# kasirershahartau/tissue_image_processing

Measured on AMD Instinct MI355X. Metric: frames/sec end-to-end (2048^2, z=30), higher is better.
Workload: dtype f32(f16x3)

## Files before the change

tissue_image_processing_amd/csrc/tip_core.hip:

```cpp
#include "tip_internal.h"
#include <algorithm>
#include <cmath>
#include <cstdlib>
#include <map>
#include <mutex>

namespace tip {

static thread_local Ctx *g_ctx = nullptr;
static thread_local int g_requested_device = 0;

static int ctx_create(int device)
{
    Ctx *c = new Ctx();
    c->device = device;
    hipError_t e = hipSetDevice(device);
    if (e != hipSuccess) {
        c->err = std::string("hipSetDevice failed: ") + hipGetErrorString(e);
        g_ctx = c;
        return TIP_ERR_HIP;
    }
    {
        const char *pr = getenv("TIP_STREAM_PRIORITY");
        int lo = 0, hi = 0;
// ... 61 lines not shown
    }
    c.pool.push_back({p, bytes, true});
    return p;
}

void *pinned_scratch(size_t bytes)
{
    Ctx &c = ctx();
    if (c.pin_bytes >= bytes && c.pin_buf) return c.pin_buf;
    if (c.pin_buf) { (void)hipHostFree(c.pin_buf); c.pin_buf = nullptr; c.pin_bytes = 0; }
    const size_t want = bytes + (bytes >> 2) + 4096;
    void *p = nullptr;
    if (hipHostMalloc(&p, want, hipHostMallocDefault) != hipSuccess) {
        (void)hipGetLastError();
        fail(TIP_ERR_NOMEM, "hipHostMalloc(%zu) failed", want);
        return nullptr;
    }
    c.pin_buf = p;
    c.pin_bytes = want;
    return p;
}

void ws_free(void *p)
{
    Ctx &c = ctx();
    for (auto &b : c.pool)
        if (b.p == p) { b.used = false; return; }
}

void prof_begin(const char *name)
{
    Ctx &c = ctx();
    if (!c.prof) return;
    ProfRec r;
    r.name = name;
    if (c.free_events.size() >= 2) {
        r.e0 = c.free_events.back(); c.free_events.pop_back();
        r.e1 = c.free_events.back(); c.free_events.pop_back();
    } else {
        (void)hipEventCreate(&r.e0);
        (void)hipEventCreate(&r.e1);
    }
    (void)hipEventRecord(r.e0, c.stream);
    c.recs.push_back(r);
}

void prof_end()
{
    Ctx &c = ctx();
    if (!c.prof) return;
    (void)hipEventRecord(c.recs.back().e1, c.stream);
}

namespace {
Tuning g_tuning;
std::once_flag g_tuning_once;
std::mutex g_tuning_mu;

bool tuning_assign(Tuning &t, const char *name, const char *value)
{
    const Tuning def;
    const bool unset = !value || !*value;
    auto flag = [&](int &field, int dflt) { field = unset ? dflt : (strcmp(value, "0") != 0 ? 1 : 0); };
    auto num = [&](int &field, int dflt) { field = unset ? dflt : atoi(value); };
    auto pair = [&](int &a, int &b, int da, int db) {
        a = da; b = db;
        if (!unset) sscanf(value, "%d,%d", &a, &b);
    };
    const std::string n(name ? name : "");
    if (n == "TIP_WS_TIES") {
        if (unset) t.ws_ties = def.ws_ties;
        else t.ws_ties = (!strcmp(value, "fast") || !strcmp(value, "0")) ? 0 : 1;
    }
    else if (n == "TIP_WS_OPEN") pair(t.ws_open_a, t.ws_open_b, def.ws_open_a, def.ws_open_b);
    else if (n == "TIP_WS_NO_SKIP") flag(t.ws_no_skip, 0);
    else if (n == "TIP_WS_DEBUG") flag(t.ws_debug, 0);
    else if (n == "TIP_WS_NO_ENDGAME") flag(t.ws_no_endgame, 0);
    else if (n == "TIP_WS_NO_WIDE") flag(t.ws_no_wide, 0);
    else if (n == "TIP_PROJECT_GENERIC") flag(t.project_generic, 0);
    else if (n == "TIP_PROJECT_UNFUSED_PREBLUR") flag(t.project_unfused_preblur, 0);
    else if (n == "TIP_PROJECT_UNFUSED_MASK") flag(t.project_unfused_mask, 0);
    else if (n == "TIP_PROJECT_EXACT_SCORE") flag(t.project_exact_score, 0);
    else if (n == "TIP_PROJECT_DEBUG") flag(t.project_debug, 0);
    else if (n == "TIP_UNET_TILE8") num(t.unet_tile8, def.unet_tile8);
    else if (n == "TIP_UF_ONE_LEVEL") flag(t.uf_one_level, 0);
    else if (n == "TIP_UNET_SPB") num(t.unet_spb, def.unet_spb);
    else if (n == "TIP_UNET_MFMA") { num(t.unet_mfma, def.unet_mfma); if (t.unet_mfma != 32) t.unet_mfma = 16; }
    else if (n == "TIP_UNET_XCD_MAP") flag(t.unet_xcd_map, 1);
    else if (n == "TIP_UNET_FIRST") {
        if (unset || !strcmp(value, "mfma")) t.unet_first_mfma = def.unet_first_mfma;
        else t.unet_first_mfma = !strcmp(value, "valu") ? 0 : std::max(atoi(value), 0);
    }
    else if (n == "TIP_UNET_TAIL_UNFUSED") flag(t.unet_tail_unfused, 0);
    else if (n == "TIP_MB_SMALL") num(t.mb_small, def.mb_small);
    else if (n == "TIP_MB_BATCH") num(t.mb_batch, def.mb_batch);
    else return false;
    return true;
}

const char *const TUNING_NAMES[] = {"TIP_WS_TIES", "TIP_WS_OPEN", "TIP_WS_NO_SKIP", "TIP_WS_DEBUG", "TIP_WS_NO_ENDGAME", "TIP_WS_NO_WIDE",
                                    "TIP_PROJECT_GENERIC", "TIP_PROJECT_UNFUSED_PREBLUR", "TIP_PROJECT_UNFUSED_MASK",
                                    "TIP_PROJECT_EXACT_SCORE", "TIP_PROJECT_DEBUG", "TIP_UNET_TILE8", "TIP_UNET_TAIL_UNFUSED", "TIP_UNET_XCD_MAP", "TIP_UNET_SPB", "TIP_UNET_MFMA", "TIP_UNET_FIRST", "TIP_UF_ONE_LEVEL", "TIP_MB_SMALL", "TIP_MB_BATCH"};

void tuning_from_env()
{
    for (const char *name : TUNING_NAMES)
        if (const char *e = getenv(name)) tuning_assign(g_tuning, name, e);
}
}

const Tuning &tuning()
{
    std::call_once(g_tuning_once, tuning_from_env);
    return g_tuning;
}

int make_taps(Taps &t, const double *w, int n)
{
    if (n <= 0 || n > 255 || !(n & 1)) return fail(TIP_ERR_ARG, "tap count %d must be odd and <= 255", n);
    for (int i = 1; i <= n / 2; i++)
        if (fabs(w[n / 2 + i] - w[n / 2 - i]) > 2.220446049250313e-16)
            return fail(TIP_ERR_UNSUPPORTED, "only symmetric kernels (scipy's symmetric correlate1d branch)");
    memset(&t, 0, sizeof t);
    for (int i = 0; i < n; i++) t.w[i] = w[i];
    t.n = n;
    return TIP_OK;
}

static double np_pairwise_sum(const double *a, long n)
{
    if (n < 8) {
        double r = 0.0;
        for (long i = 0; i < n; i++) r += a[i];
        return r;
    } else if (n <= 128) {
        double r[8];
        long i;
        for (i = 0; i < 8; i++) r[i] = a[i];
        for (i = 8; i < n - (n % 8); i += 8)
            for (int k = 0; k < 8; k++) r[k] += a[i + k];
        double res = ((r[0] + r[1]) + (r[2] + r[3])) + ((r[4] + r[5]) + (r[6] + r[7]));
        for (; i < n; i++) res += a[i];
        return res;
    }
    long n2 = n / 2;
    n2 -= n2 % 8;
    return np_pairwise_sum(a, n2) + np_pairwise_sum(a + n2, n - n2);
}

int libm_taps(double sigma, double truncate, double *w, int cap)
{
    long radius = (long)(truncate * sigma + 0.5);
    long n = 2 * radius + 1;
    if (n > cap) return -1;
    double s2 = sigma * sigma;
    for (long i = 0; i < n; i++) {
        double x = (double)(i - radius);
        w[i] = exp(-0.5 / s2 * (x * x));
    }
    double sum = np_pairwise_sum(w, n);
    for (long i = 0; i < n; i++) w[i] = w[i] / sum;
    return (int)n;
}

}

using namespace tip;

extern "C" {

int tip_version(void) { return 100; }

int tip_device_count(void)
{
    int n = 0;
    if (hipGetDeviceCount(&n) != hipSuccess) return 0;
    return n;
}

int tip_init(int device)
{
    if (g_ctx) {
        if (g_ctx->device == device && g_ctx->stream) return TIP_OK;
        tip_shutdown();
    }
// ... 190 lines not shown
```

tissue_image_processing_amd/csrc/tip_corr_f16.h:

```cpp
#pragma once
#include "tip_corr.h"
#include "tip_unet_conv.h"

namespace tip {

constexpr int HF_TO = 256, HF_LN = 32, HF_NW = 4;
typedef float hf_f32x4 __attribute__((ext_vector_type(4)));

struct HfScale {
    float s, inv;
};
__device__ __forceinline__ HfScale hf_scale(const float *clip_p95, const int *clip_has)
{
    const float c = (clip_has && *clip_has && *clip_p95 > 0.f) ? *clip_p95 : 1.f;
    const int e = min(max((int)((__float_as_uint(c) >> 23) & 0xffu) - 127, -60), 100);
    HfScale h;
    h.s = __uint_as_float((unsigned)(127 + 13 - e) << 23);
    h.inv = __uint_as_float((unsigned)(127 - 13 + e - 17) << 23);
    return h;
}

template <int AXIS, int R8>
__global__ void __launch_bounds__(HF_NW * 64, 2) k_corr_long_f16(const float *__restrict__ in, float *__restrict__ out, int Z, int Y, int X,
                                                                  TapsF taps, const float *__restrict__ clip_p95, const int *__restrict__ clip_has,
                                                                  int *__restrict__ range_flag, int tiles_ln, int tiles_pos, int xcd_bands)
{
    constexpr int r = 8 * R8, NPOS = HF_TO + 2 * r, S = R8 + 2;
    constexpr int PCH = (NPOS / 8) | 1, PITCH = PCH * 8;
    constexpr int WROWS = 2 * S + 3;
    extern __shared__ __attribute__((aligned(16))) unsigned char hf_smem[];
    _Float16 *sB_hi = reinterpret_cast<_Float16 *>(hf_smem), *sB_lo = sB_hi + HF_LN * PITCH;
    uint4 *sW_hi = reinterpret_cast<uint4 *>(sB_lo + HF_LN * PITCH), *sW_lo = sW_hi + WROWS * 8;
    const int tid = threadIdx.x, lane = tid & 63, wave = __builtin_amdgcn_readfirstlane(tid >> 6);
    const int z = blockIdx.y;
    int lx, py;
    if (AXIS == 2 && xcd_bands) {
        const int b = blockIdx.x, k = b & 7, j = b >> 3;
        py = j % tiles_pos;
        lx = k + 8 * (j / tiles_pos);
    } else {
        lx = blockIdx.x % tiles_ln;
        py = blockIdx.x / tiles_ln;
    }
    const int p0 = py * HF_TO, l0 = lx * HF_LN;
    const long P = (long)Y * X;
    const float *src = in + (long)z * P;
    const HfScale sc = hf_scale(clip_p95, clip_has);

    for (int idx = tid; idx < WROWS * 8; idx += HF_NW * 64) {
        const int up = (idx >> 3) - 3, c = idx & 7;
        f16x8 hi, lo;
#pragma unroll
        for (int e = 0; e < 8; ++e) {
            const int d = 8 * up - c + e, ad = d - r < 0 ? r - d : d - r;
            const float w = (d >= 0 && d <= 2 * r) ? taps.w[r - ad] * 131072.f : 0.f;
            hi[e] = (_Float16)w;
            lo[e] = (_Float16)((w - (float)hi[e]) * 2048.f);
        }
        sW_hi[idx] = __builtin_bit_cast(uint4, hi);
        sW_lo[idx] = __builtin_bit_cast(uint4, lo);
    }
    float vmax = 0.f;
    auto split8 = [&](const float (&v)[8], int line, int g) {
        f16x8 hi, lo;
#pragma unroll
        for (int e = 0; e < 8; ++e) {
            const float vs = v[e] * sc.s;
            vmax = fmax_raw(vmax, vs);
            hi[e] = (_Float16)vs;
            lo[e] = (_Float16)__builtin_fmaf(vs - (float)hi[e], 2048.f, fminf(vs * 1.329227995784916e36f, 5.9604644775390625e-8f));
        }
        *reinterpret_cast<uint4 *>(sB_hi + line * PITCH + 8 * g) = __builtin_bit_cast(uint4, hi);
        *reinterpret_cast<uint4 *>(sB_lo + line * PITCH + 8 * g) = __builtin_bit_cast(uint4, lo);
    };
    constexpr int NG = NPOS / 8;
    if (AXIS == 2) {
        constexpr int NIT = (HF_LN * NG + HF_NW * 64 - 1) / (HF_NW * 64);
        hf_f32x4 ld[NIT][2];
        const bool vec = (X & 3) == 0;
        constexpr int DL = (HF_NW * 64) / NG, DG = (HF_NW * 64) - DL * NG;
        const int line_0 = tid / NG, g_0 = tid - line_0 * NG;
        int uline[NIT], ug[NIT];
        {
            int line = line_0, g = g_0;
#pragma unroll
            for (int it = 0; it < NIT; ++it) {
                uline[it] = line;
                ug[it] = g;
                line += DL;
                g += DG;
                if (g >= NG) { g -= NG; ++line; }
            }
        }
#pragma unroll
        for (int it = 0; it < NIT; ++it) {
            const int line = uline[it], g = ug[it];
            const float *row = src + (long)min(l0 + min(line, HF_LN - 1), Y - 1) * X;
            const int x0 = p0 - r + 8 * g;
            if (vec && x0 >= 0 && x0 + 8 <= X) {
                ld[it][0] = *reinterpret_cast<const hf_f32x4 *>(row + x0);
                ld[it][1] = *reinterpret_cast<const hf_f32x4 *>(row + x0 + 4);
            } else {
                ld[it][0] = hf_f32x4{row[clampi(x0, 0, X - 1)], row[clampi(x0 + 1, 0, X - 1)], row[clampi(x0 + 2, 0, X - 1)], row[clampi(x0 + 3, 0, X - 1)]};
                ld[it][1] = hf_f32x4{row[clampi(x0 + 4, 0, X - 1)], row[clampi(x0 + 5, 0, X - 1)], row[clampi(x0 + 6, 0, X - 1)], row[clampi(x0 + 7, 0, X - 1)]};
            }
        }
#pragma unroll
        for (int it = 0; it < NIT; ++it) {
            const int line = uline[it], g = ug[it];
            if (line < HF_LN) {
                const float v[8] = {ld[it][0][0], ld[it][0][1], ld[it][0][2], ld[it][0][3], ld[it][1][0], ld[it][1][1], ld[it][1][2], ld[it][1][3]};
                split8(v, line, g);
            }
        }
    } else {
        constexpr int NIT = (NG * (HF_LN / 4) + HF_NW * 64 - 1) / (HF_NW * 64);
        hf_f32x4 ld[NIT][8];
        const int lq = tid & 7;
        const int xq = l0 + 4 * lq;
        const bool vec = (X & 3) == 0 && xq + 4 <= X;
        if (vec) {
#pragma unroll
            for (int it = 0; it < NIT; ++it) {
                const int g = min(it * (HF_NW * 8) + (tid >> 3), NG - 1), y0 = p0 - r + 8 * g;
#pragma unroll
                for (int e = 0; e < 8; ++e) ld[it][e] = *reinterpret_cast<const hf_f32x4 *>(src + (long)clampi(y0 + e, 0, Y - 1) * X + xq);
            }
        } else {
#pragma unroll
            for (int it = 0; it < NIT; ++it) {
                const int g = min(it * (HF_NW * 8) + (tid >> 3), NG - 1), y0 = p0 - r + 8 * g;
#pragma unroll
                for (int e = 0; e < 8; ++e) {
                    const float *row = src + (long)clampi(y0 + e, 0, Y - 1) * X;
                    ld[it][e] = hf_f32x4{row[min(xq, X - 1)], row[min(xq + 1, X - 1)], row[min(xq + 2, X - 1)], row[min(xq + 3, X - 1)]};
                }
            }
        }
#pragma unroll
        for (int it = 0; it < NIT; ++it) {
            const int g = it * (HF_NW * 8) + (tid >> 3);
            if (g < NG) {
                float v[8];
#pragma unroll
                for (int e = 0; e < 8; ++e) v[e] = ld[it][e].x;
                split8(v, 4 * lq, g);
#pragma unroll
                for (int e = 0; e < 8; ++e) v[e] = ld[it][e].y;
                split8(v, 4 * lq + 1, g);
#pragma unroll
                for (int e = 0; e < 8; ++e) v[e] = ld[it][e].z;
                split8(v, 4 * lq + 2, g);
#pragma unroll
                for (int e = 0; e < 8; ++e) v[e] = ld[it][e].w;
                split8(v, 4 * lq + 3, g);
            }
        }
    }
    if (!(vmax < 40000.f)) atomicOr(range_flag, 8);
    __syncthreads();

    const int i = lane & 31, h = lane >> 5;
    const int len = AXIS == 1 ? Y : X;
    if (p0 + wave * 64 >= len) return;
    const _Float16 *bh = sB_hi + i * PITCH + wave * 64 + 8 * h, *bl = sB_lo + i * PITCH + wave * 64 + 8 * h;
    const int wrow0 = (h - (i >> 3) + 3) * 8 + (i & 7);
    f32x16 thh[2], tm[2], ahh[2], am[2];
#pragma unroll
    for (int t = 0; t < 2; ++t)
#pragma unroll
        for (int q = 0; q < 16; ++q) { thh[t][q] = 0.f; tm[t][q] = 0.f; ahh[t][q] = 0.f; am[t][q] = 0.f; }
    uint4 fh[3], fl[3];
    auto mm = [](const uint4 &wf, const uint4 &sf, const f32x16 &c) -> f32x16 {
        if (AXIS == 1) return __builtin_amdgcn_mfma_f32_32x32x16_f16(__builtin_bit_cast(f16x8, wf), __builtin_bit_cast(f16x8, sf), c, 0, 0, 0);
        return __builtin_amdgcn_mfma_f32_32x32x16_f16(__builtin_bit_cast(f16x8, sf), __builtin_bit_cast(f16x8, wf), c, 0, 0, 0);
    };
    auto flush = [&](int t) {
#pragma unroll
        for (int q = 0; q < 16; q += 2) {
            f32x2 x = f32x2{thh[t][q], thh[t][q + 1]} + f32x2{ahh[t][q], ahh[t][q + 1]};
            f32x2 y = f32x2{tm[t][q], tm[t][q + 1]} + f32x2{am[t][q], am[t][q + 1]};
            asm volatile("" : "+v"(x), "+v"(y));
            thh[t][q] = x[0]; thh[t][q + 1] = x[1];
            tm[t][q] = y[0]; tm[t][q + 1] = y[1];
            ahh[t][q] = 0.f; ahh[t][q + 1] = 0.f;
            am[t][q] = 0.f; am[t][q + 1] = 0.f;
        }
    };
#pragma unroll
    for (int s = 0; s < S + 2; ++s) {
        const uint4 sh = *reinterpret_cast<const uint4 *>(bh + 16 * s), sl = *reinterpret_cast<const uint4 *>(bl + 16 * s);
        if (s < S) {
            fh[s % 3] = sW_hi[wrow0 + 16 * s];
            fl[s % 3] = sW_lo[wrow0 + 16 * s];
            ahh[0] = mm(fh[s % 3], sh, ahh[0]);
            am[0] = mm(fh[s % 3], sl, am[0]);
            am[0] = mm(fl[s % 3], sh, am[0]);
            if ((s & 1) == 1 || s == S - 1) flush(0);
        }
        if (s >= 2) {
            const int k = (s - 2) % 3;
            ahh[1] = mm(fh[k], sh, ahh[1]);
            am[1] = mm(fh[k], sl, am[1]);
            am[1] = mm(fl[k], sh, am[1]);
            if (((s - 2) & 1) == 1 || s == S + 1) flush(1);
        }
        __builtin_amdgcn_sched_barrier(0);
    }
    float *dst = out + (long)z * P;
#pragma unroll
    for (int t = 0; t < 2; ++t) {
        const int o0 = p0 + wave * 64 + 32 * t;
#pragma unroll
        for (int q = 0; q < 16; ++q) {
            const int rr = (q & 3) + 8 * (q >> 2) + 4 * h;
            const float val = __builtin_fmaf(tm[t][q], 4.8828125e-4f, thh[t][q]) * sc.inv;
            if (AXIS == 1) {
                const int yy = o0 + rr, xx = l0 + i;
                if (yy < Y && xx < X) dst[(long)yy * X + xx] = val;
            } else {
                const int yy = l0 + rr, xx = o0 + i;
                if (yy < Y && xx < X) dst[(long)yy * X + xx] = val;
            }
        }
    }
}

}
```

tissue_image_processing_amd/csrc/tip_internal.h:

```cpp
#pragma once
#include <hip/hip_runtime.h>
#include <cstdarg>
#include <cstdint>
#include <cstdio>
#include <cstring>
#include <string>
#include <vector>
#include "../../include/tissue_hip.h"

namespace tip {

struct ProfRec { const char *name; hipEvent_t e0, e1; };

struct Ctx {
    int device = -1;
    hipStream_t stream = nullptr;
    std::string err;
    struct Block { void *p; size_t bytes; bool used; };
    std::vector<Block> pool;
    int last_ws_labels = 0;
    long last_ws_other = 0;
    hipEvent_t edge_event = nullptr;
    void *prep_ws = nullptr;
    unsigned *unet_status = nullptr;
    int *unet_status_host = nullptr;
    void *pin_buf = nullptr;
    size_t pin_bytes = 0;
    bool prof = false;
    std::vector<ProfRec> recs;
    std::vector<hipEvent_t> free_events;
};

Ctx &ctx();
int fail(int code, const char *fmt, ...);
int launch_check(const char *what);
void *ws_alloc(size_t bytes);
void *pinned_scratch(size_t bytes);
void ws_free(void *p);

struct WsGuard {
    std::vector<void *> ptrs;
    template <typename T> T *get(size_t count) {
        void *p = ws_alloc(count * sizeof(T) ? count * sizeof(T) : 16);
        if (p) ptrs.push_back(p);
        return (T *)p;
    }
    ~WsGuard() { for (void *p : ptrs) ws_free(p); }
};

struct Staging {
    WsGuard ws;
    int rc = TIP_OK;
    struct Out { void *host; const void *dev; size_t bytes; };
    std::vector<Out> outs;

    bool hip(hipError_t e, const char *what)
    {
        if (e != hipSuccess && !rc) rc = fail(TIP_ERR_HIP, "%s failed: %s", what, hipGetErrorString(e));
        return !rc;
    }
    template <typename T> T *scratch(size_t count)
    {
        if (rc) return nullptr;
        T *d = ws.get<T>(count);
        if (!d) rc = TIP_ERR_NOMEM;
        return d;
    }
    template <typename T> T *in(const T *host, size_t count)
    {
        T *d = host ? scratch<T>(count) : nullptr;
        if (d && count) hip(hipMemcpyAsync(d, host, count * sizeof(T), hipMemcpyHostToDevice, ctx().stream), "hipMemcpyAsync (upload)");
        return d;
    }
    template <typename T> T *out(T *host, size_t count, bool zero = false)
    {
        T *d = host ? scratch<T>(count) : nullptr;
        if (d && zero && count) hip(hipMemsetAsync(d, 0, count * sizeof(T), ctx().stream), "hipMemsetAsync");
        if (d) outs.push_back({host, d, count * sizeof(T)});
        return d;
    }
    template <typename T> void set_count(const T *dev, size_t count)
    {
        for (Out &o : outs)
            if (o.dev == dev && count * sizeof(T) < o.bytes) o.bytes = count * sizeof(T);
    }
    int finish()
    {
        for (const Out &o : outs)
            if (o.bytes && !hip(hipMemcpyAsync(o.host, o.dev, o.bytes, hipMemcpyDeviceToHost, ctx().stream), "hipMemcpyAsync (download)")) break;
        if (!rc) hip(hipStreamSynchronize(ctx().stream), "hipStreamSynchronize");
        return rc;
    }
};

void prof_begin(const char *name);
void prof_end();

struct Tuning {
    int ws_ties = 1;
    int ws_open_a = -1, ws_open_b = -1;
    int ws_no_skip = 0;
    int ws_debug = 0;
    int ws_no_endgame = 0, ws_no_wide = 0;
    int project_generic = 0, project_unfused_preblur = 0, project_unfused_mask = 0;
    int project_exact_score = 0, project_debug = 0;
    int unet_tail_unfused = 0;
    int unet_xcd_map = 1;
    int unet_spb = 3;
    int unet_mfma = 32;
    int unet_first_mfma = 1;
    int uf_one_level = 0;
    int mb_small = -1;
    int mb_batch = -1;
    int unet_tile8 = -1;
};
const Tuning &tuning();

#define TIP_HIP(call)                                                                             \
    do {                                                                                          \
        hipError_t e__ = (call);                                                                  \
        if (e__ != hipSuccess)                                                                    \
            return tip::fail(TIP_ERR_HIP, "%s failed: %s (%s:%d)", #call, hipGetErrorString(e__), \
                             __FILE__, __LINE__);                                                 \
    } while (0)

#define TIP_LAUNCH(name, kernel, grid, block, shmem, ...)                                  \
    do {                                                                                   \
        tip::prof_begin(name);                                                             \
        hipLaunchKernelGGL(kernel, grid, block, shmem, tip::ctx().stream, __VA_ARGS__);    \
        tip::prof_end();                                                                   \
        hipError_t e__ = hipGetLastError();                                                \
        if (e__ != hipSuccess)                                                             \
            return tip::fail(TIP_ERR_HIP, "launch %s: %s", name, hipGetErrorString(e__));  \
    } while (0)

static inline int cdiv(long a, long b) { return (int)((a + b - 1) / b); }

struct Taps {
    double w[256];
    int n;
};
struct TapsF {
    float w[256];
    int n;
};

int make_taps(Taps &t, const double *w, int n);
int libm_taps(double sigma, double truncate, double *w, int cap);
int correlate1d_dev(const void *in, void *out, int dtype, int Z, int Y, int X, int axis, const Taps &t, int force);

constexpr int OF_F64_AS_U16 = 5;
int optical_flow_tvl1_dev(const void *ref, const void *mov, int dtype, int y, int x, float attachment, float tightness,
                          int num_warp, int num_iter, double tol, float *flow_out, int32_t *warps_host, int cap);

int scan_i32_dev(const int32_t *in, int32_t *out, int n);

}
```

tissue_image_processing_amd/csrc/tip_project.hip:

```cpp
#include "tip_slide.h"
#include "tip_preblur.h"
#include "tip_corr.h"
#include "tip_corr_f16.h"
#include "tip_manifold.h"
#include "tip_project_binned.h"
#include <algorithm>
#include <atomic>
#include <cstdlib>

namespace tip {

struct ClipInfo {
    double p95d;
    float p95;
    int has;
};

template <typename T>
__device__ __forceinline__ T wave_inclusive_scan(T v, int lane)
{
    for (int d = 1; d < 64; d <<= 1) {
        const T o = __shfl_up(v, d, 64);
        if (lane >= d) v += o;
    }
// ... 270 lines not shown
        for (int c = cx; c < cx + 8 + 2 * MASK_R; ++c) { za = min(za, (int)cmin[ty][c]); zb = max(zb, (int)cmax[ty][c]); }
        za = max(za - MASK_ZR, 0); zb = min(zb + MASK_ZR, Zs - 1);
    }
    float mx[MAXC][8];
#pragma unroll
    for (int c = 0; c < MAXC; ++c)
#pragma unroll
        for (int k = 0; k < 8; ++k) mx[c][k] = 0.f;
    for (int z = zaB; z <= zbB; ++z) {
        float(*yb)[FT_W] = ybuf[(z - zaB) & 1];
        const float *Tz = sT + z * Zs;
        for (int i = t; i < FT_Y * FT_W; i += 256) {
            const int r = i / FT_W, c = i - r * FT_W;
            float val = 0.f;
            if (z >= (int)cmin[r][c] - MASK_ZR && z <= (int)cmax[r][c] + MASK_ZR)
                val = (float)tap_sum<MASK_R>([&](int j) { return (double)Tz[zs[r + j][c]]; }, taps.w);
            yb[r][c] = val;
        }
        __syncthreads();
        if (live && z >= za && z <= zb) {
            float v[8 + 2 * MASK_R];
#pragma unroll
            for (int i = 0; i < (8 + 2 * MASK_R) / 4; ++i) {
                const float4 f = *reinterpret_cast<const float4 *>(&yb[ty][cx + 4 * i]);
                v[4 * i] = f.x; v[4 * i + 1] = f.y; v[4 * i + 2] = f.z; v[4 * i + 3] = f.w;
            }
            float m[8];
#pragma unroll
            for (int k = 0; k < 8; ++k) m[k] = (float)tap_sum<MASK_R>([&](int j) { return (double)v[k + j]; }, taps.w);
#pragma unroll
            for (int c = 0; c < MAXC; ++c) {
                if (c < C && ((chan_mask >> c) & 1u)) {
                    const uint16_t *ip = img + ((long)c * Zfull + zlo + z) * P + (long)gy * X + gx;
                    unsigned short pix[8];
                    if (gx + 8 <= X && (X & 7) == 0) {
                        const uint4 u = *reinterpret_cast<const uint4 *>(ip);
                        pix[0] = u.x & 0xffff; pix[1] = u.x >> 16; pix[2] = u.y & 0xffff; pix[3] = u.y >> 16;
                        pix[4] = u.z & 0xffff; pix[5] = u.z >> 16; pix[6] = u.w & 0xffff; pix[7] = u.w >> 16;
                    } else {
#pragma unroll
                        for (int k = 0; k < 8; ++k) pix[k] = gx + k < X ? ip[k] : 0;
                    }
#pragma unroll
                    for (int k = 0; k < 8; ++k) {
                        const float pr = airy_offset((float)pix[k], airy) * m[k];
                        mx[c][k] = pr > mx[c][k] ? pr : mx[c][k];
                    }
                }
            }
        }
    }
    if (live) {
#pragma unroll
        for (int c = 0; c < MAXC; ++c)
            if (c < C && ((chan_mask >> c) & 1u))
#pragma unroll
                for (int k = 0; k < 8; ++k)
                    if (gx + k < X) proj[(long)c * P + (long)gy * X + gx + k] = (double)mx[c][k];
    }
}

static int cu_count()
{
    static int cus = 0;
    if (!cus) {
        hipDeviceProp_t prop;
        cus = hipGetDeviceProperties(&prop, ctx().device) == hipSuccess && prop.multiProcessorCount > 0 ? prop.multiProcessorCount : 256;
    }
    return cus;
}

static TapsF taps_f32(const double *w, int n)
{
    TapsF f;
    f.n = n;
    for (int i = 0; i < 256; ++i) f.w[i] = i < n ? (float)w[i] : 0.f;
    return f;
}

template <int AXIS>
static int launch_f16(const float *in, float *out, int Zs, int Y, int X, const TapsF &t, const ClipInfo *clip, int *range_flag)
{
    if (t.n != 241 || !clip || !range_flag) return fail(TIP_ERR_ARG, "f16 score pass: %d taps (241 only) or no clip value / range flag", t.n);
    constexpr int R8 = 15, NPOS = HF_TO + 16 * R8, PITCH = ((NPOS / 8) | 1) * 8, WROWS = 2 * (R8 + 2) + 3;
    const size_t lds = (size_t)2 * HF_LN * PITCH * 2 + (size_t)2 * WROWS * 8 * 16;
    auto k = k_corr_long_f16<AXIS, R8>;
    static std::atomic<unsigned> attr_done[64];
    const int dev = ctx().device >= 0 && ctx().device < 64 ? ctx().device : 0;
    if (!(attr_done[dev].load(std::memory_order_acquire) & (1u << AXIS))) {
        TIP_HIP(hipFuncSetAttribute((const void *)k, hipFuncAttributeMaxDynamicSharedMemorySize, (int)lds));
        attr_done[dev].fetch_or(1u << AXIS, std::memory_order_release);
    }
    const int tiles_ln = cdiv(AXIS == 1 ? X : Y, HF_LN), tiles_pos = cdiv(AXIS == 1 ? Y : X, HF_TO);
    if ((long)tiles_ln * tiles_pos > 0x7fffffffL || Zs > 65535) return fail(TIP_ERR_ARG, "f16 score pass: grid too large");
    const dim3 grid((unsigned)(tiles_ln * tiles_pos), (unsigned)Zs);
    const int xcd_bands = (AXIS == 2 && tiles_ln % 8 == 0) ? 1 : 0;
    TIP_LAUNCH(AXIS == 1 ? "score_fast_y" : "score_fast_x", k, grid, dim3(HF_NW * 64), lds, in, out, Zs, Y, X, t, &clip->p95, &clip->has, range_flag,
               tiles_ln, tiles_pos, xcd_bands);
    return TIP_OK;
}

#define CERT_EPS (96.0f * 5.9604644775390625e-8f)
__device__ __forceinline__ float cert_abs(const ClipInfo *clip)
{
    return (clip && clip->has) ? clip->p95 * 5.684341886080802e-14f + 1e-30f : 1e-30f;
}

__global__ void __launch_bounds__(256) k_argmax_certify(const float *__restrict__ score, int Z, long P, int *__restrict__ best_z,
                                                        int *__restrict__ unc_list, int *__restrict__ unc_count, const ClipInfo *clip)
{
    __shared__ int s_cnt[4], s_base;
    const float dabs = cert_abs(clip);
    const long p0 = ((long)blockIdx.x * blockDim.x + threadIdx.x) * 4;
    const bool vec = p0 + 4 <= P && (P & 3) == 0;
    float b1[4], b2[4];
    int z1[4];
#pragma unroll
    for (int k = 0; k < 4; ++k) { b1[k] = -1.f; b2[k] = -1.f; z1[k] = 0; }
    if (p0 < P) {
        for (int z = 0; z < Z; ++z) {
            float v[4];
            if (vec) {
                const float4 f = *reinterpret_cast<const float4 *>(score + (long)z * P + p0);
                v[0] = f.x; v[1] = f.y; v[2] = f.z; v[3] = f.w;
            } else {
#pragma unroll
                for (int k = 0; k < 4; ++k) v[k] = p0 + k < P ? score[(long)z * P + p0 + k] : 0.f;
            }
#pragma unroll
            for (int k = 0; k < 4; ++k) {
                if (v[k] > b1[k]) { b2[k] = b1[k]; b1[k] = v[k]; z1[k] = z; }
                else if (v[k] > b2[k]) b2[k] = v[k];
            }
        }
    }
    unsigned unc = 0;
#pragma unroll
    for (int k = 0; k < 4; ++k) {
        if (p0 + k >= P) continue;
        best_z[p0 + k] = z1[k];
        const bool certain = (b1[k] == 0.f) || (Z == 1) || (b1[k] * (1.f - CERT_EPS) - dabs > b2[k] * (1.f + CERT_EPS) + dabs);
        if (!certain) unc |= 1u << k;
    }
    const int mine = __popc(unc);
    const int lane = threadIdx.x & 63, wave = threadIdx.x >> 6;
    const int incl = wave_inclusive_scan(mine, lane);
    if (lane == 63) s_cnt[wave] = incl;
    __syncthreads();
    if (threadIdx.x == 0) {
        const int tot = s_cnt[0] + s_cnt[1] + s_cnt[2] + s_cnt[3];
        s_base = tot ? atomicAdd(unc_count, tot) : 0;
    }
    __syncthreads();
    if (mine) {
        int off = s_base + incl - mine;
        for (int w = 0; w < wave; ++w) off += s_cnt[w];
#pragma unroll
        for (int k = 0; k < 4; ++k)
            if ((unc >> k) & 1u) unc_list[off++] = (int)(p0 + k);
    }
}

constexpr int FIX_UL = 16;
__global__ void __launch_bounds__(256) k_argmax_exact_fix(const float *__restrict__ zvol, const float *__restrict__ score, int Z, int Y,
                                                          int X, Taps taps, const int *__restrict__ unc_list,
                                                          const int *__restrict__ unc_count, int *__restrict__ best_z, const ClipInfo *clip)
{
    const float dabs = cert_abs(clip);
    __shared__ float c[256];
    __shared__ float sfast[64];
    __shared__ float sexact[64];
    __shared__ int s_z;
    const int r = taps.n >> 1;
    const int total = *unc_count, xcd = blockIdx.x & 7, per = (total + 7) / 8;
    for (int sl = blockIdx.x >> 3; sl < per; sl += gridDim.x >> 3) {
        const int u = xcd * per + sl;
        if (u >= total) break;
        const int p = unc_list[u];
        const int y = p / X, x = p - y * X;
        const long P = (long)Y * X;
        if (threadIdx.x < Z) sfast[threadIdx.x] = score[(long)threadIdx.x * P + p];
// ... 491 lines not shown
```

Before: 21.53.

## Walk several output tiles per block through an LDS ring buffer for halo reuse

Each block of the f16 long-correlation score pass now processes several consecutive output tiles (default 4) along the filter axis. It keeps a 512-position ring buffer in LDS, so only the new 256 positions are staged per step and the 240-tap halo is reused. The aim is to cut redundant global loads and hi/lo splitting of halo data, which was nearly half of each tile's input. In exchange the grid shrinks fourfold, reducing parallelism and per-block overlap, and extra barriers serialize staging with the MFMA compute.

Result: no change. 21.61 (median of 5 runs) (+0.4%).

```diff
diff --git a/tissue_image_processing_amd/csrc/tip_core.hip b/tissue_image_processing_amd/csrc/tip_core.hip
--- a/tissue_image_processing_amd/csrc/tip_core.hip
+++ b/tissue_image_processing_amd/csrc/tip_core.hip
@@ -167,6 +167,10 @@
     else if (n == "TIP_PROJECT_UNFUSED_MASK") flag(t.project_unfused_mask, 0);
     else if (n == "TIP_PROJECT_EXACT_SCORE") flag(t.project_exact_score, 0);
     else if (n == "TIP_PROJECT_DEBUG") flag(t.project_debug, 0);
+    else if (n == "TIP_SCORE_WALK") {
+        t.score_walk_y = t.score_walk_x = 0;
+        if (!unset && sscanf(value, "%d,%d", &t.score_walk_y, &t.score_walk_x) == 1) t.score_walk_x = t.score_walk_y;
+    }
     else if (n == "TIP_UNET_TILE8") num(t.unet_tile8, def.unet_tile8);
     else if (n == "TIP_UF_ONE_LEVEL") flag(t.uf_one_level, 0);
     else if (n == "TIP_UNET_SPB") num(t.unet_spb, def.unet_spb);
@@ -185,7 +189,7 @@
 
 const char *const TUNING_NAMES[] = {"TIP_WS_TIES", "TIP_WS_OPEN", "TIP_WS_NO_SKIP", "TIP_WS_DEBUG", "TIP_WS_NO_ENDGAME", "TIP_WS_NO_WIDE",
                                     "TIP_PROJECT_GENERIC", "TIP_PROJECT_UNFUSED_PREBLUR", "TIP_PROJECT_UNFUSED_MASK",
-                                    "TIP_PROJECT_EXACT_SCORE", "TIP_PROJECT_DEBUG", "TIP_UNET_TILE8", "TIP_UNET_TAIL_UNFUSED", "TIP_UNET_XCD_MAP", "TIP_UNET_SPB", "TIP_UNET_MFMA", "TIP_UNET_FIRST", "TIP_UF_ONE_LEVEL", "TIP_MB_SMALL", "TIP_MB_BATCH"};
+                                    "TIP_PROJECT_EXACT_SCORE", "TIP_PROJECT_DEBUG", "TIP_SCORE_WALK", "TIP_UNET_TILE8", "TIP_UNET_TAIL_UNFUSED", "TIP_UNET_XCD_MAP", "TIP_UNET_SPB", "TIP_UNET_MFMA", "TIP_UNET_FIRST", "TIP_UF_ONE_LEVEL", "TIP_MB_SMALL", "TIP_MB_BATCH"};
 
 void tuning_from_env()
 {
diff --git a/tissue_image_processing_amd/csrc/tip_corr_f16.h b/tissue_image_processing_amd/csrc/tip_corr_f16.h
--- a/tissue_image_processing_amd/csrc/tip_corr_f16.h
+++ b/tissue_image_processing_amd/csrc/tip_corr_f16.h
@@ -5,6 +5,29 @@
 namespace tip {
 
 constexpr int HF_TO = 256, HF_LN = 32, HF_NW = 4;
+constexpr int HF_RING = 512;
+constexpr int HF_PCH = HF_RING / 8 + 1, HF_PITCH = 8 * HF_PCH;
+constexpr int HF_WALK_Y = 4, HF_WALK_X = 4;
+constexpr int hf_ring_slot(int q) { return q & (HF_RING - 1); }
+struct HfWalk { int lx, py0; };
+constexpr HfWalk hf_walk_of_block(int b, bool bands, int tiles_ln, int walks_pos, int walk)
+{
+    if (bands) return HfWalk{(b & 7) + 8 * ((b >> 3) / walks_pos), ((b >> 3) % walks_pos) * walk};
+    return HfWalk{b % tiles_ln, (b / tiles_ln) * walk};
+}
+constexpr bool hf_conflict_free(int pch)
+{
+    for (int g = 0; g < 4; ++g) {
+        unsigned seen = 0;
+        for (int i = 0; i < 16; ++i) {
+            const int lane = uc_group_lane(g, i), quad = ((lane & 31) * pch + (lane >> 5)) & 15;
+            if (seen & (1u << quad)) return false;
+            seen |= 1u << quad;
+        }
+    }
+    return true;
+}
+static_assert((HF_RING & (HF_RING - 1)) == 0 && hf_conflict_free(HF_PCH), "ring length a power of two; 16 different bank quads per lane group of ds_read_b128");
 typedef float hf_f32x4 __attribute__((ext_vector_type(4)));
 
 struct HfScale {
@@ -23,26 +46,20 @@
 template <int AXIS, int R8>
 __global__ void __launch_bounds__(HF_NW * 64, 2) k_corr_long_f16(const float *__restrict__ in, float *__restrict__ out, int Z, int Y, int X,
                                                                   TapsF taps, const float *__restrict__ clip_p95, const int *__restrict__ clip_has,
-                                                                  int *__restrict__ range_flag, int tiles_ln, int tiles_pos, int xcd_bands)
+                                                                  int *__restrict__ range_flag, int tiles_ln, int tiles_pos, int xcd_bands, int walk)
 {
     constexpr int r = 8 * R8, NPOS = HF_TO + 2 * r, S = R8 + 2;
-    constexpr int PCH = (NPOS / 8) | 1, PITCH = PCH * 8;
+    constexpr int PITCH = HF_PITCH;
     constexpr int WROWS = 2 * S + 3;
+    static_assert(NPOS <= HF_RING && NPOS % 8 == 0, "a tile's positions fit the ring, in whole groups of eight");
     extern __shared__ __attribute__((aligned(16))) unsigned char hf_smem[];
     _Float16 *sB_hi = reinterpret_cast<_Float16 *>(hf_smem), *sB_lo = sB_hi + HF_LN * PITCH;
     uint4 *sW_hi = reinterpret_cast<uint4 *>(sB_lo + HF_LN * PITCH), *sW_lo = sW_hi + WROWS * 8;
     const int tid = threadIdx.x, lane = tid & 63, wave = __builtin_amdgcn_readfirstlane(tid >> 6);
     const int z = blockIdx.y;
-    int lx, py;
-    if (AXIS == 2 && xcd_bands) {
-        const int b = blockIdx.x, k = b & 7, j = b >> 3;
-        py = j % tiles_pos;
-        lx = k + 8 * (j / tiles_pos);
-    } else {
-        lx = blockIdx.x % tiles_ln;
-        py = blockIdx.x / tiles_ln;
-    }
-    const int p0 = py * HF_TO, l0 = lx * HF_LN;
+    const HfWalk wk = hf_walk_of_block(blockIdx.x, AXIS == 2 && xcd_bands, tiles_ln, (tiles_pos + walk - 1) / walk, walk);
+    const int ntiles = min(walk, tiles_pos - wk.py0);
+    const int P0 = wk.py0 * HF_TO, l0 = wk.lx * HF_LN;
     const long P = (long)Y * X;
     const float *src = in + (long)z * P;
     const HfScale sc = hf_scale(clip_p95, clip_has);
@@ -61,7 +78,7 @@
         sW_lo[idx] = __builtin_bit_cast(uint4, lo);
     }
     float vmax = 0.f;
-    auto split8 = [&](const float (&v)[8], int line, int g) {
+    auto split8 = [&](const float (&v)[8], int line, int G) {
         f16x8 hi, lo;
 #pragma unroll
         for (int e = 0; e < 8; ++e) {
@@ -70,160 +87,175 @@
             hi[e] = (_Float16)vs;
             lo[e] = (_Float16)__builtin_fmaf(vs - (float)hi[e], 2048.f, fminf(vs * 1.329227995784916e36f, 5.9604644775390625e-8f));
         }
-        *reinterpret_cast<uint4 *>(sB_hi + line * PITCH + 8 * g) = __builtin_bit_cast(uint4, hi);
-        *reinterpret_cast<uint4 *>(sB_lo + line * PITCH + 8 * g) = __builtin_bit_cast(uint4, lo);
+        const int slot = line * PITCH + hf_ring_slot(8 * G);
+        *reinterpret_cast<uint4 *>(sB_hi + slot) = __builtin_bit_cast(uint4, hi);
+        *reinterpret_cast<uint4 *>(sB_lo + slot) = __builtin_bit_cast(uint4, lo);
     };
-    constexpr int NG = NPOS / 8;
-    if (AXIS == 2) {
-        constexpr int NIT = (HF_LN * NG + HF_NW * 64 - 1) / (HF_NW * 64);
-        hf_f32x4 ld[NIT][2];
-        const bool vec = (X & 3) == 0;
-        constexpr int DL = (HF_NW * 64) / NG, DG = (HF_NW * 64) - DL * NG;
-        const int line_0 = tid / NG, g_0 = tid - line_0 * NG;
-        int uline[NIT], ug[NIT];
-        {
-            int line = line_0, g = g_0;
+    constexpr int NG = NPOS / 8, NG_NEXT = HF_TO / 8;
+    auto stage = [&](int G0, auto ngrp) {
+        constexpr int NGRP = decltype(ngrp)::value;
+        if (AXIS == 2) {
+            constexpr int NIT = (HF_LN * NGRP + HF_NW * 64 - 1) / (HF_NW * 64);
+            hf_f32x4 ld[NIT][2];
+            const bool vec = (X & 3) == 0;
+            constexpr int DL = (HF_NW * 64) / NGRP, DG = (HF_NW * 64) - DL * NGRP;
+            const int line_0 = tid / NGRP, g_0 = tid - line_0 * NGRP;
+            int uline[NIT], ug[NIT];
+            {
+                int line = line_0, g = g_0;
+#pragma unroll
+                for (int it = 0; it < NIT; ++it) {
+                    uline[it] = line;
+                    ug[it] = g;
+                    line += DL;
+                    g += DG;
+                    if (g >= NGRP) { g -= NGRP; ++line; }
+                }
+            }
 #pragma unroll
             for (int it = 0; it < NIT; ++it) {
-                uline[it] = line;
-                ug[it] = g;
-                line += DL;
-                g += DG;
-                if (g >= NG) { g -= NG; ++line; }
-            }
-        }
-#pragma unroll
-        for (int it = 0; it < NIT; ++it) {
-            const int line = uline[it], g = ug[it];
-            const float *row = src + (long)min(l0 + min(line, HF_LN - 1), Y - 1) * X;
-            const int x0 = p0 - r + 8 * g;
-            if (vec && x0 >= 0 && x0 + 8 <= X) {
-                ld[it][0] = *reinterpret_cast<const hf_f32x4 *>(row + x0);
-                ld[it][1] = *reinterpret_cast<const hf_f32x4 *>(row + x0 + 4);
+                const int line = uline[it], g = ug[it];
+                const float *row = src + (long)min(l0 + min(line, HF_LN - 1), Y - 1) * X;
+                const int x0 = P0 - r + 8 * (G0 + g);
+                if (vec && x0 >= 0 && x0 + 8 <= X) {
+                    ld[it][0] = *reinterpret_cast<const hf_f32x4 *>(row + x0);
+                    ld[it][1] = *reinterpret_cast<const hf_f32x4 *>(row + x0 + 4);
+                } else {
+                    ld[it][0] = hf_f32x4{row[clampi(x0, 0, X - 1)], row[clampi(x0 + 1, 0, X - 1)], row[clampi(x0 + 2, 0, X - 1)], row[clampi(x0 + 3, 0, X - 1)]};
+                    ld[it][1] = hf_f32x4{row[clampi(x0 + 4, 0, X - 1)], row[clampi(x0 + 5, 0, X - 1)], row[clampi(x0 + 6, 0, X - 1)], row[clampi(x0 + 7, 0, X - 1)]};
+                }
+            }
+#pragma unroll
+            for (int it = 0; it < NIT; ++it) {
+                const int line = uline[it], g = ug[it];
+                if (line < HF_LN) {
+                    const float v[8] = {ld[it][0][0], ld[it][0][1], ld[it][0][2], ld[it][0][3], ld[it][1][0], ld[it][1][1], ld[it][1][2], ld[it][1][3]};
+                    split8(v, line, G0 + g);
+                }
+            }
+        } else {
+            constexpr int NIT = (NGRP * (HF_LN / 4) + HF_NW * 64 - 1) / (HF_NW * 64);
+            hf_f32x4 ld[NIT][8];
+            const int lq = tid & 7;
+            const int xq = l0 + 4 * lq;
+            const bool vec = (X & 3) == 0 && xq + 4 <= X;
+            if (vec) {
+#pragma unroll
+                for (int it = 0; it < NIT; ++it) {
+                    const int g = min(it * (HF_NW * 8) + (tid >> 3), NGRP - 1), y0 = P0 - r + 8 * (G0 + g);
+#pragma unroll
+                    for (int e = 0; e < 8; ++e) ld[it][e] = *reinterpret_cast<const hf_f32x4 *>(src + (long)clampi(y0 + e, 0, Y - 1) * X + xq);
+                }
             } else {
-                ld[it][0] = hf_f32x4{row[clampi(x0, 0, X - 1)], row[clampi(x0 + 1, 0, X - 1)], row[clampi(x0 + 2, 0, X - 1)], row[clampi(x0 + 3, 0, X - 1)]};
-                ld[it][1] = hf_f32x4{row[clampi(x0 + 4, 0, X - 1)], row[clampi(x0 + 5, 0, X - 1)], row[clampi(x0 + 6, 0, X - 1)], row[clampi(x0 + 7, 0, X - 1)]};
-            }
-        }
-#pragma unroll
-        for (int it = 0; it < NIT; ++it) {
-            const int line = uline[it], g = ug[it];
-            if (line < HF_LN) {
-                const float v[8] = {ld[it][0][0], ld[it][0][1], ld[it][0][2], ld[it][0][3], ld[it][1][0], ld[it][1][1], ld[it][1][2], ld[it][1][3]};
-                split8(v, line, g);
-            }
-        }
-    } else {
-        constexpr int NIT = (NG * (HF_LN / 4) + HF_NW * 64 - 1) / (HF_NW * 64);
-        hf_f32x4 ld[NIT][8];
-        const int lq = tid & 7;
-        const int xq = l0 + 4 * lq;
-        const bool vec = (X & 3) == 0 && xq + 4 <= X;
-        if (vec) {
+#pragma unroll
+                for (int it = 0; it < NIT; ++it) {
+                    const int g = min(it * (HF_NW * 8) + (tid >> 3), NGRP - 1), y0 = P0 - r + 8 * (G0 + g);
+#pragma unroll
+                    for (int e = 0; e < 8; ++e) {
+                        const float *row = src + (long)clampi(y0 + e, 0, Y - 1) * X;
+                        ld[it][e] = hf_f32x4{row[min(xq, X - 1)], row[min(xq + 1, X - 1)], row[min(xq + 2, X - 1)], row[min(xq + 3, X - 1)]};
+                    }
+                }
+            }
 #pragma unroll
             for (int it = 0; it < NIT; ++it) {
-                const int g = min(it * (HF_NW * 8) + (tid >> 3), NG - 1), y0 = p0 - r + 8 * g;
-#pragma unroll
-                for (int e = 0; e < 8; ++e) ld[it][e] = *reinterpret_cast<const hf_f32x4 *>(src + (long)clampi(y0 + e, 0, Y - 1) * X + xq);
-            }
-        } else {
-#pragma unroll
-            for (int it = 0; it < NIT; ++it) {
-                const int g = min(it * (HF_NW * 8) + (tid >> 3), NG - 1), y0 = p0 - r + 8 * g;
-#pragma unroll
-                for (int e = 0; e < 8; ++e) {
-                    const float *row = src + (long)clampi(y0 + e, 0, Y - 1) * X;
-                    ld[it][e] = hf_f32x4{row[min(xq, X - 1)], row[min(xq + 1, X - 1)], row[min(xq + 2, X - 1)], row[min(xq + 3, X - 1)]};
-                }
-            }
-        }
-#pragma unroll
-        for (int it = 0; it < NIT; ++it) {
-            const int g = it * (HF_NW * 8) + (tid >> 3);
-            if (g < NG) {
-                float v[8];
-#pragma unroll
-                for (int e = 0; e < 8; ++e) v[e] = ld[it][e].x;
-                split8(v, 4 * lq, g);
-#pragma unroll
-                for (int e = 0; e < 8; ++e) v[e] = ld[it][e].y;
-                split8(v, 4 * lq + 1, g);
-#pragma unroll
-                for (int e = 0; e < 8; ++e) v[e] = ld[it][e].z;
-                split8(v, 4 * lq + 2, g);
-#pragma unroll
-                for (int e = 0; e < 8; ++e) v[e] = ld[it][e].w;
-                split8(v, 4 * lq + 3, g);
-            }
-        }
-    }
-    if (!(vmax < 40000.f)) atomicOr(range_flag, 8);
-    __syncthreads();
+                const int g = it * (HF_NW * 8) + (tid >> 3);
+                if (g < NGRP) {
+                    float v[8];
+#pragma unroll
+                    for (int e = 0; e < 8; ++e) v[e] = ld[it][e].x;
+                    split8(v, 4 * lq, G0 + g);
+#pragma unroll
+                    for (int e = 0; e < 8; ++e) v[e] = ld[it][e].y;
+                    split8(v, 4 * lq + 1, G0 + g);
+#pragma unroll
+                    for (int e = 0; e < 8; ++e) v[e] = ld[it][e].z;
+                    split8(v, 4 * lq + 2, G0 + g);
+#pragma unroll
+                    for (int e = 0; e < 8; ++e) v[e] = ld[it][e].w;
+                    split8(v, 4 * lq + 3, G0 + g);
+                }
+            }
+        }
+    };
 
     const int i = lane & 31, h = lane >> 5;
     const int len = AXIS == 1 ? Y : X;
-    if (p0 + wave * 64 >= len) return;
-    const _Float16 *bh = sB_hi + i * PITCH + wave * 64 + 8 * h, *bl = sB_lo + i * PITCH + wave * 64 + 8 * h;
+    const _Float16 *bh = sB_hi + i * PITCH + 8 * h, *bl = sB_lo + i * PITCH + 8 * h;
     const int wrow0 = (h - (i >> 3) + 3) * 8 + (i & 7);
-    f32x16 thh[2], tm[2], ahh[2], am[2];
-#pragma unroll
-    for (int t = 0; t < 2; ++t)
-#pragma unroll
-        for (int q = 0; q < 16; ++q) { thh[t][q] = 0.f; tm[t][q] = 0.f; ahh[t][q] = 0.f; am[t][q] = 0.f; }
-    uint4 fh[3], fl[3];
     auto mm = [](const uint4 &wf, const uint4 &sf, const f32x16 &c) -> f32x16 {
         if (AXIS == 1) return __builtin_amdgcn_mfma_f32_32x32x16_f16(__builtin_bit_cast(f16x8, wf), __builtin_bit_cast(f16x8, sf), c, 0, 0, 0);
         return __builtin_amdgcn_mfma_f32_32x32x16_f16(__builtin_bit_cast(f16x8, sf), __builtin_bit_cast(f16x8, wf), c, 0, 0, 0);
     };
-    auto flush = [&](int t) {
-#pragma unroll
-        for (int q = 0; q < 16; q += 2) {
-            f32x2 x = f32x2{thh[t][q], thh[t][q + 1]} + f32x2{ahh[t][q], ahh[t][q + 1]};
-            f32x2 y = f32x2{tm[t][q], tm[t][q + 1]} + f32x2{am[t][q], am[t][q + 1]};
-            asm volatile("" : "+v"(x), "+v"(y));
-            thh[t][q] = x[0]; thh[t][q + 1] = x[1];
-            tm[t][q] = y[0]; tm[t][q + 1] = y[1];
-            ahh[t][q] = 0.f; ahh[t][q + 1] = 0.f;
-            am[t][q] = 0.f; am[t][q + 1] = 0.f;
-        }
-    };
-#pragma unroll
-    for (int s = 0; s < S + 2; ++s) {
-        const uint4 sh = *reinterpret_cast<const uint4 *>(bh + 16 * s), sl = *reinterpret_cast<const uint4 *>(bl + 16 * s);
-        if (s < S) {
-            fh[s % 3] = sW_hi[wrow0 + 16 * s];
-            fl[s % 3] = sW_lo[wrow0 + 16 * s];
-            ahh[0] = mm(fh[s % 3], sh, ahh[0]);
-            am[0] = mm(fh[s % 3], sl, am[0]);
-            am[0] = mm(fl[s % 3], sh, am[0]);
-            if ((s & 1) == 1 || s == S - 1) flush(0);
-        }
-        if (s >= 2) {
-            const int k = (s - 2) % 3;
-            ahh[1] = mm(fh[k], sh, ahh[1]);
-            am[1] = mm(fh[k], sl, am[1]);
-            am[1] = mm(fl[k], sh, am[1]);
-            if (((s - 2) & 1) == 1 || s == S + 1) flush(1);
-        }
-        __builtin_amdgcn_sched_barrier(0);
+    float *dst = out + (long)z * P;
+    stage(0, std::integral_constant<int, NG>());
+    for (int k = 0; k < ntiles; ++k) {
+        __syncthreads();
+        const int p0 = P0 + k * HF_TO;
+        if (p0 + wave * 64 < len) {
+            const int q0 = k * HF_TO + wave * 64;
+            f32x16 thh[2], tm[2], ahh[2], am[2];
+#pragma unroll
+            for (int t = 0; t < 2; ++t)
+#pragma unroll
+                for (int q = 0; q < 16; ++q) { thh[t][q] = 0.f; tm[t][q] = 0.f; ahh[t][q] = 0.f; am[t][q] = 0.f; }
+            uint4 fh[3], fl[3];
+            auto flush = [&](int t) {
+#pragma unroll
+                for (int q = 0; q < 16; q += 2) {
+                    f32x2 x = f32x2{thh[t][q], thh[t][q + 1]} + f32x2{ahh[t][q], ahh[t][q + 1]};
+                    f32x2 y = f32x2{tm[t][q], tm[t][q + 1]} + f32x2{am[t][q], am[t][q + 1]};
+                    asm volatile("" : "+v"(x), "+v"(y));
+                    thh[t][q] = x[0]; thh[t][q + 1] = x[1];
+                    tm[t][q] = y[0]; tm[t][q + 1] = y[1];
+                    ahh[t][q] = 0.f; ahh[t][q + 1] = 0.f;
+                    am[t][q] = 0.f; am[t][q + 1] = 0.f;
+                }
+            };
+#pragma unroll
+            for (int s = 0; s < S + 2; ++s) {
+                const int slot = hf_ring_slot(q0 + 16 * s);
+                const uint4 sh = *reinterpret_cast<const uint4 *>(bh + slot), sl = *reinterpret_cast<const uint4 *>(bl + slot);
+                if (s < S) {
+                    fh[s % 3] = sW_hi[wrow0 + 16 * s];
+                    fl[s % 3] = sW_lo[wrow0 + 16 * s];
+                    ahh[0] = mm(fh[s % 3], sh, ahh[0]);
+                    am[0] = mm(fh[s % 3], sl, am[0]);
+                    am[0] = mm(fl[s % 3], sh, am[0]);
+                    if ((s & 1) == 1 || s == S - 1) flush(0);
+                }
+                if (s >= 2) {
+                    const int kk = (s - 2) % 3;
+                    ahh[1] = mm(fh[kk], sh, ahh[1]);
+                    am[1] = mm(fh[kk], sl, am[1]);
+                    am[1] = mm(fl[kk], sh, am[1]);
+                    if (((s - 2) & 1) == 1 || s == S + 1) flush(1);
+                }
+                __builtin_amdgcn_sched_barrier(0);
+            }
+#pragma unroll
+            for (int t = 0; t < 2; ++t) {
+                const int o0 = p0 + wave * 64 + 32 * t;
+#pragma unroll
+                for (int q = 0; q < 16; ++q) {
+                    const int rr = (q & 3) + 8 * (q >> 2) + 4 * h;
+                    const float val = __builtin_fmaf(tm[t][q], 4.8828125e-4f, thh[t][q]) * sc.inv;
+                    if (AXIS == 1) {
+                        const int yy = o0 + rr, xx = l0 + i;
+                        if (yy < Y && xx < X) dst[(long)yy * X + xx] = val;
+                    } else {
+                        const int yy = l0 + rr, xx = o0 + i;
+                        if (yy < Y && xx < X) dst[(long)yy * X + xx] = val;
+                    }
+                }
+            }
+        }
+        if (k + 1 < ntiles) {
+            __syncthreads();
+            stage(NG + NG_NEXT * k, std::integral_constant<int, NG_NEXT>());
+        }
     }
-    float *dst = out + (long)z * P;
-#pragma unroll
-    for (int t = 0; t < 2; ++t) {
-        const int o0 = p0 + wave * 64 + 32 * t;
-#pragma unroll
-        for (int q = 0; q < 16; ++q) {
-            const int rr = (q & 3) + 8 * (q >> 2) + 4 * h;
-            const float val = __builtin_fmaf(tm[t][q], 4.8828125e-4f, thh[t][q]) * sc.inv;
-            if (AXIS == 1) {
-                const int yy = o0 + rr, xx = l0 + i;
-                if (yy < Y && xx < X) dst[(long)yy * X + xx] = val;
-            } else {
-                const int yy = l0 + rr, xx = o0 + i;
-                if (yy < Y && xx < X) dst[(long)yy * X + xx] = val;
-            }
-        }
-    }
-}
-
-}
+    if (!(vmax < 40000.f)) atomicOr(range_flag, 8);
+}
+
+}
diff --git a/tissue_image_processing_amd/csrc/tip_internal.h b/tissue_image_processing_amd/csrc/tip_internal.h
--- a/tissue_image_processing_amd/csrc/tip_internal.h
+++ b/tissue_image_processing_amd/csrc/tip_internal.h
@@ -104,6 +104,7 @@
     int ws_no_endgame = 0, ws_no_wide = 0;
     int project_generic = 0, project_unfused_preblur = 0, project_unfused_mask = 0;
     int project_exact_score = 0, project_debug = 0;
+    int score_walk_y = 0, score_walk_x = 0;
     int unet_tail_unfused = 0;
     int unet_xcd_map = 1;
     int unet_spb = 3;
diff --git a/tissue_image_processing_amd/csrc/tip_project.hip b/tissue_image_processing_amd/csrc/tip_project.hip
--- a/tissue_image_processing_amd/csrc/tip_project.hip
+++ b/tissue_image_processing_amd/csrc/tip_project.hip
@@ -376,8 +376,8 @@
 static int launch_f16(const float *in, float *out, int Zs, int Y, int X, const TapsF &t, const ClipInfo *clip, int *range_flag)
 {
     if (t.n != 241 || !clip || !range_flag) return fail(TIP_ERR_ARG, "f16 score pass: %d taps (241 only) or no clip value / range flag", t.n);
-    constexpr int R8 = 15, NPOS = HF_TO + 16 * R8, PITCH = ((NPOS / 8) | 1) * 8, WROWS = 2 * (R8 + 2) + 3;
-    const size_t lds = (size_t)2 * HF_LN * PITCH * 2 + (size_t)2 * WROWS * 8 * 16;
+    constexpr int R8 = 15, WROWS = 2 * (R8 + 2) + 3;
+    const size_t lds = (size_t)2 * HF_LN * HF_PITCH * 2 + (size_t)2 * WROWS * 8 * 16;
     auto k = k_corr_long_f16<AXIS, R8>;
     static std::atomic<unsigned> attr_done[64];
     const int dev = ctx().device >= 0 && ctx().device < 64 ? ctx().device : 0;
@@ -387,10 +387,12 @@
     }
     const int tiles_ln = cdiv(AXIS == 1 ? X : Y, HF_LN), tiles_pos = cdiv(AXIS == 1 ? Y : X, HF_TO);
     if ((long)tiles_ln * tiles_pos > 0x7fffffffL || Zs > 65535) return fail(TIP_ERR_ARG, "f16 score pass: grid too large");
-    const dim3 grid((unsigned)(tiles_ln * tiles_pos), (unsigned)Zs);
+    const int tuned = AXIS == 1 ? tuning().score_walk_y : tuning().score_walk_x;
+    const int walk = std::min(tuned > 0 ? tuned : (AXIS == 1 ? HF_WALK_Y : HF_WALK_X), tiles_pos);
+    const dim3 grid((unsigned)(tiles_ln * cdiv(tiles_pos, walk)), (unsigned)Zs);
     const int xcd_bands = (AXIS == 2 && tiles_ln % 8 == 0) ? 1 : 0;
     TIP_LAUNCH(AXIS == 1 ? "score_fast_y" : "score_fast_x", k, grid, dim3(HF_NW * 64), lds, in, out, Zs, Y, X, t, &clip->p95, &clip->has, range_flag,
-               tiles_ln, tiles_pos, xcd_bands);
+               tiles_ln, tiles_pos, xcd_bands, walk);
     return TIP_OK;
 }
 
```
